# hwang595/ps_pytorch

Measured on AMD Instinct MI355X. Metric: images/sec (whole node), ResNet-18/CIFAR-10 synchronous PS training, higher is better.
Workload: dtype bf16; 1 GPU; model=ResNet18, global_batch=1024, input=3x32x32, per_worker_batch=1024, parallelism=single-gpu, engine=single-machine trainer (hipGraph-captured step), compress_grad=n/a (no comm at N=1), overlap=n/a (no comm at N=1)

## Files before the change

ps_pytorch_amd/ops/__init__.py:

```python
from __future__ import annotations

import ctypes
import os
from pathlib import Path
from typing import Optional

import torch

_LIB: Optional[ctypes.CDLL] = None
_LIB_ERR: Optional[str] = None

PS_F32 = 0
PS_BF16 = 1

_DTYPE_TAG = {torch.float32: PS_F32, torch.bfloat16: PS_BF16}

F32_SYMBOLS = (
    'ps_conv_fwd_f32', 'ps_conv_dgrad_f32', 'ps_conv_wgrad_f32',
    'ps_conv_bias_grad_f32',
    'ps_maxpool_fwd_f32', 'ps_maxpool_bwd_f32',
    'ps_gavgpool_fwd_f32', 'ps_gavgpool_bwd_f32',
    'ps_softmax_ce_fwd_f32', 'ps_softmax_ce_bwd_f32',
    'ps_ce_metrics_f32', 'ps_softmax_ce_fwd_metrics_f32',
)


def _so_path() -> Path:
    return Path(__file__).resolve().parent / "libps_hip.so"


def _try_load() -> None:
    global _LIB, _LIB_ERR
    if _LIB is not None or _LIB_ERR is not None:
        return
    p = _so_path()
    if not p.exists():
        _LIB_ERR = f"{p} not built (run ps_pytorch_amd.ops.build or __graft_entry__.build())"
        return
    try:
        lib = ctypes.CDLL(str(p))
        lib.ps_fused_sgd.argtypes = [
            ctypes.c_void_p, ctypes.c_void_p, ctypes.c_void_p, ctypes.c_void_p,
            ctypes.c_long, ctypes.c_float, ctypes.c_float, ctypes.c_float,
            ctypes.c_float, ctypes.c_int, ctypes.c_int, ctypes.c_int, ctypes.c_void_p]
        lib.ps_pack_bf16.argtypes = [ctypes.c_void_p, ctypes.c_void_p,
                                     ctypes.c_long, ctypes.c_void_p]
        lib.ps_unpack_bf16.argtypes = [ctypes.c_void_p, ctypes.c_void_p,
                                       ctypes.c_long, ctypes.c_void_p]
        lib.ps_pack_q8.argtypes = [ctypes.c_void_p, ctypes.c_void_p,
                                   ctypes.c_long, ctypes.c_int, ctypes.c_void_p]
        lib.ps_pack_q8_ef.argtypes = [ctypes.c_void_p, ctypes.c_void_p,
                                      ctypes.c_void_p, ctypes.c_long,
                                      ctypes.c_int, ctypes.c_void_p]
        lib.ps_pack_bf16_ef.argtypes = [ctypes.c_void_p, ctypes.c_void_p,
                                        ctypes.c_void_p, ctypes.c_long,
                                        ctypes.c_void_p]
        lib.ps_unpack_q8.argtypes = [ctypes.c_void_p, ctypes.c_void_p,
                                     ctypes.c_long, ctypes.c_int, ctypes.c_void_p]
        lib.ps_acc.argtypes = [ctypes.c_void_p, ctypes.c_void_p,
                               ctypes.c_long, ctypes.c_int, ctypes.c_void_p]
        lib.ps_pack_topk_ef.argtypes = [ctypes.c_void_p] * 3 + [
            ctypes.c_long, ctypes.c_int, ctypes.c_int, ctypes.c_void_p]
        lib.ps_pack_topk_ef.restype = ctypes.c_int
        lib.ps_unpack_topk.argtypes = [ctypes.c_void_p, ctypes.c_void_p,
                                       ctypes.c_long, ctypes.c_int,
                                       ctypes.c_int, ctypes.c_void_p]
        lib.ps_unpack_topk.restype = ctypes.c_int
        lib.ps_fanin_reduce.argtypes = [
            ctypes.c_void_p, ctypes.POINTER(ctypes.c_void_p), ctypes.c_int,
            ctypes.c_int, ctypes.c_int, ctypes.c_long, ctypes.c_void_p]
        lib.ps_fanin_reduce.restype = ctypes.c_int
        lib.ps_fanin_sgd.argtypes = [ctypes.c_void_p] * 3 + [
            ctypes.c_int, ctypes.POINTER(ctypes.c_void_p), ctypes.c_int,
            ctypes.c_int, ctypes.c_int, ctypes.c_long] + [
            ctypes.c_float] * 4 + [ctypes.c_int, ctypes.c_void_p]
        lib.ps_fanin_sgd.restype = ctypes.c_int
        lib.ps_conv_fwd.argtypes = [ctypes.c_void_p] * 5 + [ctypes.c_int] * 11 + [ctypes.c_void_p]
        lib.ps_conv_dgrad.argtypes = [ctypes.c_void_p] * 4 + [ctypes.c_int] * 11 + [ctypes.c_void_p]
        lib.ps_conv_wgrad.argtypes = [ctypes.c_void_p] * 4 + [ctypes.c_int] * 12 + [ctypes.c_void_p]
        lib.ps_conv_bias_grad.argtypes = [ctypes.c_void_p] * 3 + [
            ctypes.c_long, ctypes.c_int, ctypes.c_void_p]
        lib.ps_wt_transpose.argtypes = [ctypes.c_void_p, ctypes.c_void_p,
                                        ctypes.c_int, ctypes.c_int, ctypes.c_void_p]
        lib.ps_fused_adam.argtypes = [ctypes.c_void_p] * 6 + [
            ctypes.c_long] + [ctypes.c_float] * 7 + [
            ctypes.c_int, ctypes.c_int, ctypes.c_void_p]
        lib.ps_bn_fwd.argtypes = [ctypes.c_void_p] * 13 + [
            ctypes.c_int,
            ctypes.c_long, ctypes.c_long, ctypes.c_float, ctypes.c_float,
            ctypes.c_int, ctypes.c_int, ctypes.c_int, ctypes.c_void_p]
        lib.ps_bn_bwd.argtypes = [ctypes.c_void_p] * 12 + [
            ctypes.c_long, ctypes.c_long, ctypes.c_int, ctypes.c_int,
            ctypes.c_void_p]
        lib.ps_softmax_ce_fwd.argtypes = [ctypes.c_void_p] * 5 + [
            ctypes.c_long, ctypes.c_int, ctypes.c_void_p]
        lib.ps_softmax_ce_bwd.argtypes = [ctypes.c_void_p] * 5 + [
            ctypes.c_long, ctypes.c_int, ctypes.c_void_p]
        lib.ps_ce_metrics.argtypes = [ctypes.c_void_p] * 5 + [
            ctypes.c_long] + [ctypes.c_int] * 6 + [ctypes.c_void_p]
        lib.ps_softmax_ce_fwd_metrics.argtypes = [ctypes.c_void_p] * 7 + [
            ctypes.c_long] + [ctypes.c_int] * 6 + [ctypes.c_void_p]
        lib.ps_maxpool_fwd.argtypes = [ctypes.c_void_p] * 3 + [
            ctypes.c_int] * 10 + [ctypes.c_void_p]
        lib.ps_maxpool_bwd.argtypes = [ctypes.c_void_p] * 3 + [
            ctypes.c_int] * 10 + [ctypes.c_void_p]
        lib.ps_gavgpool_fwd.argtypes = [ctypes.c_void_p] * 2 + [
            ctypes.c_int] * 3 + [ctypes.c_void_p]
        lib.ps_gavgpool_bwd.argtypes = [ctypes.c_void_p] * 2 + [
            ctypes.c_int] * 3 + [ctypes.c_void_p]
        lib.ps_pad4.argtypes = [ctypes.c_void_p, ctypes.c_void_p,
                                ctypes.c_long, ctypes.c_int, ctypes.c_void_p]
        lib.ps_padc.argtypes = [ctypes.c_void_p, ctypes.c_void_p,
                                ctypes.c_long, ctypes.c_int, ctypes.c_int,
                                ctypes.c_void_p]
        lib.ps_act_drop_fwd.argtypes = [ctypes.c_void_p] * 3 + [
            ctypes.c_long, ctypes.c_int, ctypes.c_int, ctypes.c_uint32,
            ctypes.c_float, ctypes.c_uint64, ctypes.c_uint32,
            ctypes.c_void_p, ctypes.c_void_p]
        lib.ps_act_drop_bwd.argtypes = [ctypes.c_void_p] * 3 + [
            ctypes.c_long, ctypes.c_int, ctypes.c_float, ctypes.c_void_p]
        lib.ps_rng_advance.argtypes = [ctypes.c_void_p, ctypes.c_void_p]
        lib.ps_augment_batch.argtypes = [ctypes.c_void_p] * 5 + [
            ctypes.c_long] + [ctypes.c_int] * 7 + [
            ctypes.POINTER(ctypes.c_float), ctypes.POINTER(ctypes.c_float),
            ctypes.c_uint64, ctypes.c_uint32, ctypes.c_void_p,
            ctypes.c_void_p]
        lib.ps_conv_fwd_f32.argtypes = [ctypes.c_void_p] * 4 + [ctypes.c_int] * 11 + [ctypes.c_void_p]
        lib.ps_conv_dgrad_f32.argtypes = [ctypes.c_void_p] * 4 + [ctypes.c_int] * 11 + [ctypes.c_void_p]
        lib.ps_conv_wgrad_f32.argtypes = [ctypes.c_void_p] * 4 + [ctypes.c_int] * 12 + [ctypes.c_void_p]
        lib.ps_conv_bias_grad_f32.argtypes = [ctypes.c_void_p] * 3 + [
            ctypes.c_long, ctypes.c_int, ctypes.c_void_p]
        lib.ps_softmax_ce_fwd_f32.argtypes = lib.ps_softmax_ce_fwd.argtypes
        lib.ps_softmax_ce_bwd_f32.argtypes = lib.ps_softmax_ce_bwd.argtypes
        lib.ps_ce_metrics_f32.argtypes = lib.ps_ce_metrics.argtypes
        lib.ps_softmax_ce_fwd_metrics_f32.argtypes = \
            lib.ps_softmax_ce_fwd_metrics.argtypes
        lib.ps_maxpool_fwd_f32.argtypes = lib.ps_maxpool_fwd.argtypes
        lib.ps_maxpool_bwd_f32.argtypes = lib.ps_maxpool_bwd.argtypes
        lib.ps_gavgpool_fwd_f32.argtypes = lib.ps_gavgpool_fwd.argtypes
        lib.ps_gavgpool_bwd_f32.argtypes = lib.ps_gavgpool_bwd.argtypes
        _LIB = lib
    except OSError as e:
        _LIB_ERR = str(e)


def lib_or_none() -> Optional[ctypes.CDLL]:
    _try_load()
    return _LIB


def require_lib() -> ctypes.CDLL:
    _try_load()
    if _LIB is None:
        raise RuntimeError(
            f"ps_pytorch_amd HIP extension unavailable on a GPU host: {_LIB_ERR}")
    return _LIB


def dtype_tag(dt: torch.dtype) -> int:
    try:
        return _DTYPE_TAG[dt]
    except KeyError:
        raise TypeError(f"unsupported wire/compute dtype {dt}")


def current_stream_ptr() -> int:
    return torch.cuda.current_stream().cuda_stream


from . import functional
```

ps_pytorch_amd/ops/kernels/conv.hip:

```cpp
#include "common.h"
#include <stdlib.h>

typedef __bf16 bf16x8_t __attribute__((ext_vector_type(8)));
typedef unsigned short ushort8_t __attribute__((ext_vector_type(8)));
typedef float f32x4_t __attribute__((ext_vector_type(4)));

#define MFMA_BF16(a, b, c) __builtin_amdgcn_mfma_f32_16x16x32_bf16(a, b, c, 0, 0, 0)

union V16 {
    uint4 u4;
    unsigned short us[8];
    bf16x8_t bv;
};

__device__ __forceinline__ V16 zero16() {
    V16 v; v.u4 = make_uint4(0, 0, 0, 0); return v;
}

template <bool AL>
__device__ __forceinline__ V16 load16(const unsigned short* src, int cc, int Cn) {
    V16 v;
    if constexpr (AL) {
        v.u4 = *(const uint4*)src;
    } else if (cc + 8 <= Cn) {
// ... 932 lines not shown
    long l = (long)(blockIdx.x & 7) * per_xcd + (blockIdx.x >> 3);
    const long nlog = (long)tiles_k * tiles_c * 3 * split;
    if (l >= nlog) return;
    int b = (int)l;
    const int k0 = (b % tiles_k) * TK; b /= tiles_k;
    const int c0 = (b % tiles_c) * 64; b /= tiles_c;
    const int r = b % 3; b /= 3;
    const int sid = b;
    const long rows_total = (long)Nb * P;
    const long row0 = (long)sid * ipr;
    const long row1 = (row0 + ipr < rows_total) ? row0 + ipr : rows_total;

    const int t = threadIdx.x;
    const int cc8 = (t & 7) * 8;
    const int lane = t & 63, wid = t >> 6;
    const int wm = wid >> 1, wn = wid & 1;
    const int fr = lane & 15, fq = lane >> 4;
    f32x4_t acc[3][MI][2];
#pragma unroll
    for (int s = 0; s < 3; ++s)
#pragma unroll
        for (int i = 0; i < MI; ++i)
#pragma unroll
            for (int j = 0; j < 2; ++j) acc[s][i][j] = {0.f, 0.f, 0.f, 0.f};

    const int nsteps = (int)((row1 - row0 + (1 << (5 - l2q)) - 1)
                             >> (5 - l2q));

    const unsigned short* pdout = dout + (row0 << l2q) * K + k0 + cc8;
    const long inrow0 = row0 + r - PAD;
    const unsigned short* pin = in + inrow0 * W * C + c0 + cc8;
    long prow = row0;

    const int nbq = ROWS * HW2;
    int tb_rib[5], tb_j[5];
    bool tb_ex[5];
    bool tb_v[5];
    long tb_off[5];
#pragma unroll
    for (int u = 0; u < 5; ++u) {
        int idx = (t >> 3) + 32 * u;
        tb_ex[u] = idx < nbq;
        int ix = tb_ex[u] ? idx : 0;
        tb_rib[u] = ix / HW2; tb_j[u] = ix % HW2;
        int wpx = tb_j[u] - 1;
        tb_v[u] = tb_ex[u] && wpx >= 0 && wpx < W;
        tb_off[u] = ((long)tb_rib[u] * W + (wpx < 0 ? 0 : wpx)) * C;
    }
    V16 aregs[TK / 64], bregs[5];

    auto load_step = [&]() {
        bool mrow_ok = (prow + ((t >> 3) >> l2q)) < rows_total;
#pragma unroll
        for (int h = 0; h < TK / 64; ++h)
            aregs[h] = mrow_ok
                ? load16<AL>(pdout + (long)(t >> 3) * K + h * 64,
                             k0 + h * 64 + cc8, K)
                : zero16();
#pragma unroll
        for (int u = 0; u < 5; ++u) {
            int rib = tb_rib[u];
            int p = (int)((prow + rib) & (P - 1));
            int h = p + r - PAD;
            bool v = tb_v[u] && h >= 0 && h < H
                     && (prow + rib) < rows_total;
            bregs[u] = v ? load16<AL>(pin + tb_off[u], c0 + cc8, C)
                         : zero16();
        }
        pdout += (long)32 * K;
        pin += (long)ROWS * W * C;
        prow += ROWS;
    };

    constexpr unsigned A1 = sizeof(lds.A[0]);
    constexpr unsigned BB1 = sizeof(lds.B[0]);
    unsigned short* wrA[TK / 64];
#pragma unroll
    for (int h = 0; h < TK / 64; ++h) {
        int kk8 = h * 64 + cc8;
        wrA[h] = &lds.A[0][kk8 >> 4][pswz(t >> 3) * 16 + (kk8 & 15)];
    }
    unsigned short* wrB[5];
#pragma unroll
    for (int u = 0; u < 5; ++u) {
        int hp = pswz(tb_rib[u] * HW2 + tb_j[u]);
        wrB[u] = &lds.B[0][cc8 >> 4][hp * 16 + (cc8 & 15)];
    }

    auto write_lds = [&](int buf) {
#pragma unroll
        for (int h = 0; h < TK / 64; ++h)
            *(uint4*)((char*)wrA[h] + (buf ? A1 : 0)) = aregs[h].u4;
#pragma unroll
        for (int u = 0; u < 5; ++u)
            if (tb_ex[u])
                *(uint4*)((char*)wrB[u] + (buf ? BB1 : 0)) = bregs[u].u4;
    };

    const char* lb = (const char*)&lds;
    unsigned roA[MI][2];
    unsigned roB[3][2][2];
#pragma unroll
    for (int i = 0; i < 2; ++i) {
        int e = fq * 8 + i * 4 + (fr >> 2);
        int qo = (fr & 3) * 4;
#pragma unroll
        for (int mi = 0; mi < MI; ++mi)
            roA[mi][i] = (unsigned)((char*)&lds.A[0][wm * MI + mi]
                                    [pswz(e) * 16 + qo] - lb);
        int rib = e >> l2q, q = e & (Q - 1);
#pragma unroll
        for (int s = 0; s < 3; ++s) {
            int hp = pswz(rib * HW2 + q + s);
#pragma unroll
            for (int nj = 0; nj < 2; ++nj)
                roB[s][nj][i] = (unsigned)((char*)&lds.B[0][wn * 2 + nj]
                                           [hp * 16 + qo] - lb);
        }
    }

    union U64x8 { bf16x4_t h[2]; bf16x8_t v; };
    auto mfma_step = [&](int buf) {
        U64x8 a[MI];
#pragma unroll
        for (int mi = 0; mi < MI; ++mi) {
            a[mi].h[0] = ds_tr16p((const unsigned short*)
                (lb + roA[mi][0] + (buf ? A1 : 0)));
            a[mi].h[1] = ds_tr16p((const unsigned short*)
                (lb + roA[mi][1] + (buf ? A1 : 0)));
        }
#pragma unroll
        for (int s = 0; s < 3; ++s) {
            U64x8 bf[2];
#pragma unroll
            for (int nj = 0; nj < 2; ++nj) {
                bf[nj].h[0] = ds_tr16p((const unsigned short*)
                    (lb + roB[s][nj][0] + (buf ? BB1 : 0)));
                bf[nj].h[1] = ds_tr16p((const unsigned short*)
                    (lb + roB[s][nj][1] + (buf ? BB1 : 0)));
            }
#pragma unroll
            for (int mi = 0; mi < MI; ++mi)
#pragma unroll
                for (int nj = 0; nj < 2; ++nj)
                    acc[s][mi][nj] = MFMA_BF16(a[mi].v, bf[nj].v,
                                               acc[s][mi][nj]);
        }
    };

    load_step();
    write_lds(0);
    if (nsteps > 1) load_step();
    __syncthreads();
    for (int it = 0; it < nsteps; it += 2) {
        if (it + 1 < nsteps) {
            write_lds(1);
            if (it + 2 < nsteps) load_step();
        }
        mfma_step(0);
        __syncthreads();
        if (it + 1 >= nsteps) break;
        if (it + 2 < nsteps) {
            write_lds(0);
            if (it + 3 < nsteps) load_step();
        }
        mfma_step(1);
        __syncthreads();
    }

    const int RSC = 9 * C;
    float* dstp = partial + (long)sid * K * RSC;
#pragma unroll
    for (int s = 0; s < 3; ++s)
#pragma unroll
    for (int mi = 0; mi < MI; ++mi)
#pragma unroll
    for (int nj = 0; nj < 2; ++nj)
#pragma unroll
    for (int e = 0; e < 4; ++e) {
        int k = k0 + wm * (MI * 16) + mi * 16 + fq * 4 + e;
        int c = c0 + wn * 32 + nj * 16 + fr;
        if (k < K && c < C)
            dstp[(long)k * RSC + (r * 3 + s) * C + c] = acc[s][mi][nj][e];
    }
}


__device__ __forceinline__ int wrho(int e) {
    return (((e >> 1) & 1) + ((e >> 3) & 1) * 2) << 1;
}

template <bool AL>
__global__ __launch_bounds__(256) void conv_wgrad_row_glds_kernel(
    const unsigned short* __restrict__ dout,
    const unsigned short* __restrict__ in,
    float* __restrict__ partial,
    const unsigned short* __restrict__ zpage,
    int Nb, int H, int W, int C, int K, int P, int Q,
    int split, int ipr, int l2q, int l2p, int per_xcd)
{
    constexpr int TK = 64;
    constexpr int PAD = 1;
    const int ROWS = 32 >> l2q;
    const int HW2 = W + 2;
    __shared__ __attribute__((aligned(16))) struct {
        unsigned short A[2][32][64];
        unsigned short B[2][64][64];
    } lds;
    constexpr unsigned A1 = sizeof(lds.A[0]);
    constexpr unsigned BB1 = sizeof(lds.B[0]);
    constexpr int MI = TK / 32;
    const int tiles_k = (K + TK - 1) / TK;
    const int tiles_c = (C + 63) >> 6;
    long l = (long)(blockIdx.x & 7) * per_xcd + (blockIdx.x >> 3);
    const long nlog = (long)tiles_k * tiles_c * 3 * split;
    if (l >= nlog) return;
    int b = (int)l;
    const int k0 = (b % tiles_k) * TK; b /= tiles_k;
    const int c0 = (b % tiles_c) * 64; b /= tiles_c;
    const int r = b % 3; b /= 3;
    const int sid = b;
    const long rows_total = (long)Nb * P;
    const long row0 = (long)sid * ipr;
    const long row1 = (row0 + ipr < rows_total) ? row0 + ipr : rows_total;

    const int t = threadIdx.x;
    const int lane = t & 63, wid = t >> 6;
    const int wm = wid >> 1, wn = wid & 1;
    const int fr = lane & 15, fq = lane >> 4;
    f32x4_t acc[3][MI][2];
#pragma unroll
    for (int si = 0; si < 3; ++si)
#pragma unroll
        for (int i = 0; i < MI; ++i)
#pragma unroll
            for (int j = 0; j < 2; ++j) acc[si][i][j] = {0.f, 0.f, 0.f, 0.f};

    const int nsteps = (int)((row1 - row0 + (1 << (5 - l2q)) - 1)
                             >> (5 - l2q));

    const int apix = wid * 8 + (lane >> 3);
    const int aoct = ((lane & 7) ^ wrho(apix));
    const unsigned short* pdout = dout + (row0 << l2q) * K + k0
                                  + (long)apix * K + aoct * 8;
    const long inrow0 = row0 + r - PAD;
    const unsigned short* pin0 = in + inrow0 * W * C + c0;
    int b_rib[2], b_w[2], b_oct[2];
    bool b_wok[2];
#pragma unroll
    for (int j = 0; j < 2; ++j) {
        int hp = wid * 16 + j * 8 + (lane >> 3);
        b_oct[j] = ((lane & 7) ^ wrho(hp));
        b_rib[j] = hp / HW2;
        int wpx = hp - b_rib[j] * HW2 - 1;
        b_wok[j] = wpx >= 0 && wpx < W && hp < ROWS * HW2;
        b_w[j] = wpx < 0 ? 0 : wpx;
    }
    long prow = row0;

    auto glds_stage = [&](int buf) {
        {
            bool ok = (prow + (apix >> l2q)) < rows_total && apix < 32;
            const unsigned short* gsrc = ok ? pdout : zpage;
            __builtin_amdgcn_global_load_lds(
                (const __attribute__((address_space(1))) void*)gsrc,
                (__attribute__((address_space(3))) void*)
                    &lds.A[buf][wid * 8][0], 16, 0, 0);
        }
#pragma unroll
        for (int j = 0; j < 2; ++j) {
            int rib = b_rib[j];
            int p = (int)((prow + rib) & (P - 1));
            int h = p + r - PAD;
            bool ok = b_wok[j] && h >= 0 && h < H
                      && (prow + rib) < rows_total;
            const unsigned short* gsrc = ok
                ? pin0 + ((long)rib * W + b_w[j]) * C + b_oct[j] * 8
                : zpage;
            __builtin_amdgcn_global_load_lds(
                (const __attribute__((address_space(1))) void*)gsrc,
                (__attribute__((address_space(3))) void*)
                    &lds.B[buf][wid * 16 + j * 8][0], 16, 0, 0);
        }
        pdout += (long)32 * K;
        pin0 += (long)ROWS * W * C;
        prow += ROWS;
    };

    const char* lb0 = (const char*)&lds;
    unsigned roA[MI][2];
    unsigned roB[3][2][2];
#pragma unroll
    for (int i = 0; i < 2; ++i) {
        int e = fq * 8 + i * 4 + (fr >> 2);
        int qd = fr & 3;
#pragma unroll
        for (int mi = 0; mi < MI; ++mi) {
            int o = (wm * MI + mi) * 2 + (qd >> 1);
            roA[mi][i] = (unsigned)((char*)&lds.A[0][e]
                             [(o ^ wrho(e)) * 8 + (qd & 1) * 4] - lb0);
        }
        int rib = e >> l2q, q = e & (Q - 1);
#pragma unroll
        for (int si = 0; si < 3; ++si) {
            int hp = rib * HW2 + q + si;
#pragma unroll
            for (int nj = 0; nj < 2; ++nj) {
                int o = (wn * 2 + nj) * 2 + (qd >> 1);
                roB[si][nj][i] = (unsigned)((char*)&lds.B[0][hp]
                                 [(o ^ wrho(hp)) * 8 + (qd & 1) * 4] - lb0);
            }
        }
    }

    union U64x8 { bf16x4_t h[2]; bf16x8_t v; };
    auto mfma_step = [&](int buf) {
        U64x8 a[MI];
#pragma unroll
        for (int mi = 0; mi < MI; ++mi) {
            a[mi].h[0] = ds_tr16p((const unsigned short*)
                (lb0 + roA[mi][0] + (buf ? A1 : 0)));
            a[mi].h[1] = ds_tr16p((const unsigned short*)
                (lb0 + roA[mi][1] + (buf ? A1 : 0)));
        }
#pragma unroll
        for (int si = 0; si < 3; ++si) {
            U64x8 bf[2];
#pragma unroll
            for (int nj = 0; nj < 2; ++nj) {
                bf[nj].h[0] = ds_tr16p((const unsigned short*)
                    (lb0 + roB[si][nj][0] + (buf ? BB1 : 0)));
                bf[nj].h[1] = ds_tr16p((const unsigned short*)
                    (lb0 + roB[si][nj][1] + (buf ? BB1 : 0)));
            }
#pragma unroll
            for (int mi = 0; mi < MI; ++mi)
#pragma unroll
                for (int nj = 0; nj < 2; ++nj)
                    acc[si][mi][nj] = MFMA_BF16(a[mi].v, bf[nj].v,
                                                acc[si][mi][nj]);
        }
    };

    glds_stage(0);
    __syncthreads();
    for (int it = 0; it < nsteps; ++it) {
        if (it + 1 < nsteps)
            glds_stage((it + 1) & 1);
        mfma_step(it & 1);
        __syncthreads();
    }

    const int RSC = 9 * C;
    float* dstp = partial + (long)sid * K * RSC;
#pragma unroll
    for (int si = 0; si < 3; ++si)
#pragma unroll
    for (int mi = 0; mi < MI; ++mi)
#pragma unroll
    for (int nj = 0; nj < 2; ++nj)
#pragma unroll
    for (int e = 0; e < 4; ++e) {
        int k = k0 + wm * (MI * 16) + mi * 16 + fq * 4 + e;
        int c = c0 + wn * 32 + nj * 16 + fr;
        if (k < K && c < C)
            dstp[(long)k * RSC + (r * 3 + si) * C + c] = acc[si][mi][nj][e];
    }
}

template <int STRIDE, bool POW2, bool AL = true, int CPM = 0>
__global__ __launch_bounds__(256) void conv_wgrad_small_kernel(
    const unsigned short* __restrict__ dout,
    const unsigned short* __restrict__ in,
    float* __restrict__ partial,
    int Nb, int H, int W, int C, int K, int P, int Q,
    int R, int S, int pad, int split, int chunk,
    int l2pq, int l2q,
    unsigned long long mpq, unsigned long long mq)
{
    __shared__ __attribute__((aligned(16))) WgradLds<64> lds;
    const long M = (long)Nb * P * Q;
    const int RSC = R * S * C;
    const int tiles_k = (K + 63) >> 6;
    const int nc = (RSC + 63) >> 6;
    int b = blockIdx.x;
    const int k0 = (b % tiles_k) * 64; b /= tiles_k;
    const int e0 = (b % nc) * 64; b /= nc;
    const int sid = b;
    const long mbeg = (long)sid * chunk;
    const long mend = (mbeg + chunk < M) ? mbeg + chunk : M;

    const int t = threadIdx.x;
    const int trow = t >> 3;
    const int cc8 = (t & 7) * 8;
    const int lane = t & 63, wid = t >> 6;
    const int wm = wid >> 1, wn = wid & 1;
    const int fr = lane & 15, fq = lane >> 4;
    f32x4_t acc[2][2];
#pragma unroll
    for (int i = 0; i < 2; ++i)
#pragma unroll
        for (int j = 0; j < 2; ++j) acc[i][j] = {0.f, 0.f, 0.f, 0.f};

    int tre[8], tse[8], toff[8];
#pragma unroll
    for (int u = 0; u < 8; ++u) {
        int e = e0 + cc8 + u;
        if constexpr (CPM == 8) {
            int tp = e / C;
            tre[u] = tp / S;
            tse[u] = tp - tre[u] * S;
            toff[u] = (tre[u] * W + tse[u]) * C + (e - tp * C);
        } else if constexpr (CPM == 4) {
            int tp = e >> 2;
            tre[u] = tp / S;
            tse[u] = tp - tre[u] * S;
            toff[u] = (tre[u] * W + tse[u]) * 4;
        } else {
            tre[u] = e / (S * C);
            tse[u] = (e / C) % S;
            toff[u] = (tre[u] * W + tse[u]) * C + e % C;
        }
    }

    const int nsteps = (int)((mend - mbeg + 63) >> 6);
    long lm = mbeg;
    V16 areg[2], breg[2];

    auto load_step = [&]() {
#pragma unroll
        for (int rr = 0; rr < 2; ++rr) {
            long m = lm + trow + 32 * rr;
            V16 av = zero16(), bv = zero16();
            if (m < mend) {
                int n, p, q;
                if constexpr (POW2) {
                    n = (int)(m >> l2pq);
                    int rem = (int)m & ((1 << l2pq) - 1);
                    p = rem >> l2q; q = rem & ((1 << l2q) - 1);
                } else {
                    n = (int)fdiv_u32((unsigned)m, mpq);
                    unsigned rem = (unsigned)m - (unsigned)n * (unsigned)(P * Q);
                    p = (int)fdiv_u32(rem, mq);
                    q = (int)(rem - (unsigned)p * (unsigned)Q);
                }
                av = load16<AL>(dout + m * K + k0 + cc8, k0 + cc8, K);
                int h0 = p * STRIDE - pad, w0 = q * STRIDE - pad;
                const unsigned short* pix =
                    in + (long)n * H * W * C + ((long)h0 * W + w0) * C;
                if constexpr (CPM == 8) {
                    int hh = h0 + tre[0], ww = w0 + tse[0];
                    if (e0 + cc8 < RSC
                        && hh >= 0 && hh < H && ww >= 0 && ww < W)
                        bv.u4 = *(const uint4*)(pix + toff[0]);
                } else if constexpr (CPM == 4) {
#pragma unroll
                    for (int half = 0; half < 2; ++half) {
                        int u = 4 * half;
                        int hh = h0 + tre[u], ww = w0 + tse[u];
                        if (e0 + cc8 + u < RSC
                            && hh >= 0 && hh < H && ww >= 0 && ww < W)
                            *(unsigned long long*)&bv.us[u] =
                                *(const unsigned long long*)(pix + toff[u]);
                    }
                } else {
#pragma unroll
                for (int u = 0; u < 8; ++u) {
                    int hh = h0 + tre[u], ww = w0 + tse[u];
                    if (e0 + cc8 + u < RSC
                        && hh >= 0 && hh < H && ww >= 0 && ww < W)
                        bv.us[u] = pix[toff[u]];
                }
                }
            }
            areg[rr] = av; breg[rr] = bv;
        }
        lm += 64;
    };

    constexpr unsigned A1 = 4 * WG_SUB * 2;
    constexpr unsigned BB1 = A1;
    unsigned short* wrA[2];
    unsigned short* wrB[2];
#pragma unroll
    for (int rr = 0; rr < 2; ++rr) {
        int midx = pswz(trow + 32 * rr);
        wrA[rr] = &lds.A[0][cc8 >> 4][midx * 16 + (cc8 & 15)];
        wrB[rr] = &lds.B[0][cc8 >> 4][midx * 16 + (cc8 & 15)];
    }
    unsigned roA[2][2][2];
    unsigned roB[2][2][2];
#pragma unroll
    for (int kk = 0; kk < 2; ++kk)
#pragma unroll
        for (int i = 0; i < 2; ++i) {
            int m = pswz(kk * 32 + fq * 8 + i * 4 + (fr >> 2));
            int qo = (fr & 3) * 4;
#pragma unroll
            for (int mi = 0; mi < 2; ++mi)
                roA[kk][mi][i] = (unsigned)((char*)&lds.A[0][wm * 2 + mi]
                                            [m * 16 + qo] - (char*)&lds);
#pragma unroll
            for (int nj = 0; nj < 2; ++nj)
// ... 316 lines not shown
        int Nout_ = DG ? C : K;                                               \
        long grid = ((M_ + TM - 1) / TM) * ((Nout_ + TN - 1) / TN);           \
        hipLaunchKernelGGL((conv_gemm_kernel<TM, TN, ST, DG, SM, ALV, NBV,    \
                                             SWV, ACV, 0, GLV, STV>),         \
            dim3((unsigned)grid), dim3(256), 0, (hipStream_t)strm,            \
            (const unsigned short*)src, (const unsigned short*)wgt,           \
            (const unsigned short*)bias, (unsigned short*)dst,                \
            (const unsigned short*)carry, zpage_ptr(), (float*)stats,         \
            Nb, H, W, C, K, P, Q, R, S, pad);                                 \
    } while (0)
#define LAUNCH_GEMM_GL(TM, TN, ST, DG, SM, NBV, SWV, ACV, GLV)                \
    do {                                                                      \
        if (!(DG) && stats) LAUNCH_GEMM_GLS(TM, TN, ST, DG, SM, NBV, SWV, ACV, GLV, true); \
        else                LAUNCH_GEMM_GLS(TM, TN, ST, DG, SM, NBV, SWV, ACV, GLV, false); \
    } while (0)
#define LAUNCH_GEMM_SW(TM, TN, ST, DG, SM, NBV, SWV, ACV)                     \
    do {                                                                      \
        if constexpr (ALV && !(SM)) {                                         \
            if (glds_mode()) LAUNCH_GEMM_GL(TM, TN, ST, DG, SM, NBV, SWV, ACV, true); \
            else             LAUNCH_GEMM_GL(TM, TN, ST, DG, SM, NBV, SWV, ACV, false); \
        } else {                                                              \
            LAUNCH_GEMM_GL(TM, TN, ST, DG, SM, NBV, SWV, ACV, false);         \
        }                                                                     \
    } while (0)

extern "C" void ps_conv_fwd(
    const void* src, const void* wgt, const void* bias, void* dst,
    void* stats,
    int Nb, int H, int W, int C, int K, int P, int Q,
    int R, int S, int stride, int pad, void* strm)
{
    const void* carry = nullptr;
    bool al = (C & 63) == 0;
#define FWD_BODY()                                                            \
    do {                                                                      \
        if (R * S > 1 && C == 4 && R * S * 4 <= 64) {        \
            if (K <= 32) {            \
                if (stride == 1) LAUNCH_GEMM_CV(128, 32, 1, true, 1);         \
                else             LAUNCH_GEMM_CV(128, 32, 2, true, 1);         \
            } else if (stride == 1) LAUNCH_GEMM_CV(128, 64, 1, true, 1);      \
            else             LAUNCH_GEMM_CV(128, 64, 2, true, 1);             \
        } else if (R * S > 1 && C == 4 && R * S * 4 <= 256) {                 \
            if (K <= 32) {                                                    \
                if (stride == 1) LAUNCH_GEMM_CV(128, 32, 1, true, 2);         \
                else             LAUNCH_GEMM_CV(128, 32, 2, true, 2);         \
            } else if (stride == 1) LAUNCH_GEMM_CV(128, 64, 1, true, 2);      \
            else             LAUNCH_GEMM_CV(128, 64, 2, true, 2);             \
        } else if (R * S > 1 && (C & 7) == 0 && (C & 63)                      \
                   && R * S * C <= 768) {              \
            if (K <= 32) {                                                    \
                if (stride == 1) LAUNCH_GEMM_CP(128, 32, 1, true, 2, 8);      \
                else             LAUNCH_GEMM_CP(128, 32, 2, true, 2, 8);      \
            } else if (stride == 1) LAUNCH_GEMM_CP(128, 64, 1, true, 2, 8);   \
            else             LAUNCH_GEMM_CP(128, 64, 2, true, 2, 8);          \
        } else if (R * S > 1 && R * S * C <= 64) {    \
            if (stride == 1) LAUNCH_GEMM_NB(128, 64, 1, false, true, 1);      \
            else             LAUNCH_GEMM_NB(128, 64, 2, false, true, 1);      \
        } else if (R * S > 1 && R * S * C <= 192) {                           \
            if (stride == 1) LAUNCH_GEMM(128, 64, 1, false, true);            \
            else             LAUNCH_GEMM(128, 64, 2, false, true);            \
        } else if (R * S == 1 && C <= 64) {              \
            if (stride == 1) LAUNCH_GEMM_NB(128, 64, 1, false, false, 1);     \
            else             LAUNCH_GEMM_NB(128, 64, 2, false, false, 1);     \
        } else if (K >= 128) {                                                \
            if (stride == 1) LAUNCH_GEMM(128, 128, 1, false, false);          \
            else             LAUNCH_GEMM(128, 128, 2, false, false);          \
        } else if (K <= 32) {         \
            if (stride == 1) LAUNCH_GEMM(128, 32, 1, false, false);           \
            else             LAUNCH_GEMM(128, 32, 2, false, false);           \
        } else {                                                              \
            if (stride == 1) LAUNCH_GEMM(128, 64, 1, false, false);           \
            else             LAUNCH_GEMM(128, 64, 2, false, false);           \
        }                                                                     \
    } while (0)
    if (al) { constexpr bool ALV = true; FWD_BODY(); }
    else    { constexpr bool ALV = false; FWD_BODY(); }
#undef FWD_BODY
}

extern "C" void ps_conv_dgrad(
    const void* src, const void* wgt, void* dst, const void* carry,
    int Nb, int H, int W, int C, int K, int P, int Q,
    int R, int S, int stride, int pad, void* strm)
{
    const void* bias = nullptr;
    const void* stats = nullptr;
    bool al = (K & 63) == 0;
    if (stride == 1) {
#define DG_BODY(ACV)                                                          \
        do {                                                                  \
            if (C >= 128)     LAUNCH_GEMM_ACC(128, 128, 1, true, false, ACV); \
            else if (C <= 32) LAUNCH_GEMM_ACC(128, 32, 1, true, false, ACV);  \
            else              LAUNCH_GEMM_ACC(128, 64, 1, true, false, ACV);  \
        } while (0)
        if (al) { constexpr bool ALV = true;
                  if (carry) DG_BODY(true); else DG_BODY(false); }
        else    { constexpr bool ALV = false;
                  if (carry) DG_BODY(true); else DG_BODY(false); }
#undef DG_BODY
    } else {
        const unsigned short* dout = (const unsigned short*)src;
        bool any_empty = false;
        for (int hp = 0; hp < 2 && hp < H; ++hp)
        for (int wp = 0; wp < 2 && wp < W; ++wp) {
            int r0 = (hp + pad) & 1, s0 = (wp + pad) & 1;
            if (R <= r0 || S <= s0) any_empty = true;
        }
        if (any_empty)
            launch_seed_dx(dst, carry, (long)Nb * H * W * C, strm);
        int TM_ = 128, TN_ = (C >= 128) ? 128 : 64;
        int tiles_n_ = (C + TN_ - 1) / TN_;
        int ends_[4] = {0, 0, 0, 0}, codes_[4] = {0, 0, 0, 0};
        int slot = 0, total = 0;
        for (int hp = 0; hp < 2 && hp < H; ++hp)
        for (int wp = 0; wp < 2 && wp < W; ++wp) {
            int r0 = (hp + pad) & 1, s0 = (wp + pad) & 1;
            if (R <= r0 || S <= s0) continue;
            int Hc = (H - hp + 1) >> 1, Wc = (W - wp + 1) >> 1;
            long M_ = (long)Nb * Hc * Wc;
            total += (int)(((M_ + TM_ - 1) / TM_) * tiles_n_);
            ends_[slot] = total;
            codes_[slot] = (hp << 1) | wp;
            ++slot;
        }
        for (int i = slot; i < 4; ++i) { ends_[i] = total; codes_[i] = 0; }
        if (total == 0) return;
        int4 ends = make_int4(ends_[0], ends_[1], ends_[2], ends_[3]);
        int4 codes = make_int4(codes_[0], codes_[1], codes_[2], codes_[3]);
#define DG2_SW(TM, TN, ALV, SWV, ACV)                                         \
        hipLaunchKernelGGL((conv_dgrad2_kernel<TM, TN, ALV, SWV, ACV>),       \
            dim3((unsigned)total), dim3(256), 0, (hipStream_t)strm, dout,     \
            (const unsigned short*)wgt, (unsigned short*)dst,                 \
            (const unsigned short*)carry,                                     \
            Nb, H, W, C, K, P, Q, R, S, pad, ends, codes)
#define DG2_AC(TM, TN, ALV, SWV) do {                                         \
        if (carry) DG2_SW(TM, TN, ALV, SWV, true);                            \
        else       DG2_SW(TM, TN, ALV, SWV, false); } while (0)
#define DG2(TM, TN, ALV) do {                                                 \
        if (swz_mode() == 1) DG2_AC(TM, TN, ALV, 1);                          \
        else                 DG2_AC(TM, TN, ALV, 2); } while (0)
        if (al) { if (C >= 128) DG2(128, 128, true);
                  else          DG2(128, 64, true); }
        else    { if (C >= 128) DG2(128, 128, false);
                  else          DG2(128, 64, false); }
#undef DG2
    }
}

static inline int ilog2_exact(long v) {
    int l = 0; while ((1L << l) < v) ++l;
    return ((1L << l) == v) ? l : -1;
}

extern "C" void ps_conv_wgrad(
    const void* dout, const void* in, void* partial_f32, void* dw,
    int Nb, int H, int W, int C, int K, int P, int Q,
    int R, int S, int stride, int pad, int split, void* strm)
{
    long M = (long)Nb * P * Q;
    long chunk64 = (M + (long)split * 64 - 1) / ((long)split * 64);
    int chunk = (int)(chunk64 * 64);
    if (R * S > 1 && ((C == 4 && R * S * 4 <= 256)
                      || ((C & 7) == 0 && (C & 63) && R * S * C <= 768)
                      || R * S * C <= 192)) {
        int tiles_k = (K + 63) / 64;
        int nc_s = (R * S * C + 63) / 64;
        long grid_s = (long)tiles_k * nc_s * split;
        int l2pq_ = ilog2_exact((long)P * Q), l2q_ = ilog2_exact(Q);
        bool pw = l2pq_ >= 0 && l2q_ >= 0;
        unsigned long long mpq_ = fdiv_magic((long)P * Q);
        unsigned long long mq_ = fdiv_magic(Q);
#define WGS(ST, PW, CV)                                                       \
        hipLaunchKernelGGL((conv_wgrad_small_kernel<ST, PW, false, CV>),      \
            dim3((unsigned)grid_s), dim3(256), 0, (hipStream_t)strm,          \
            (const unsigned short*)dout, (const unsigned short*)in,           \
            (float*)partial_f32, Nb, H, W, C, K, P, Q, R, S, pad, split,      \
            chunk, l2pq_, l2q_, mpq_, mq_)
        if (C == 4) {
            if (stride == 1) { if (pw) WGS(1, true, 4); else WGS(1, false, 4); }
            else             { if (pw) WGS(2, true, 4); else WGS(2, false, 4); }
        } else if ((C & 7) == 0 && (C & 63)) {
            if (stride == 1) { if (pw) WGS(1, true, 8); else WGS(1, false, 8); }
            else             { if (pw) WGS(2, true, 8); else WGS(2, false, 8); }
        } else {
            if (stride == 1) { if (pw) WGS(1, true, 0); else WGS(1, false, 0); }
            else             { if (pw) WGS(2, true, 0); else WGS(2, false, 0); }
        }
#undef WGS
        long n_ = (long)K * R * S * C;
        launch_reduce_slabs((unsigned short*)dw, (float*)partial_f32, n_,
                            split, (hipStream_t)strm);
        return;
    }
    {
        static int row_en = -1;
        if (row_en < 0) row_en = getenv("PS_WG_ROW_OFF") ? 0 : 1;
        int l2q_ = ilog2_exact(Q), l2pq_ = ilog2_exact((long)P * Q);
        if (row_en && stride == 1 && R == 3 && S == 3 && pad == 1 && P == H
            && Q == W && l2q_ >= 0 && l2pq_ >= 0 && Q >= 4 && Q <= 32) {
            static int wg_glds = -1;
            if (wg_glds < 0) {
                const char* e = getenv("PS_WG_GLDS");
                wg_glds = e ? atoi(e) : 0;
            }
            const int TKr = 64;
            int tkr = (K + TKr - 1) / TKr, tcr = (C + 63) / 64;
            long rows_total = (long)Nb * P;
            int ROWS = 32 >> l2q_;
            long ipr_l = (rows_total + split - 1) / split;
            ipr_l = ((ipr_l + ROWS - 1) / ROWS) * ROWS;
            long nlog = (long)tkr * tcr * 3 * split;
            int pxc = (int)((nlog + 7) / 8);
            long grid_r = (long)pxc * 8;
            bool alr = ((C & 63) == 0) && (K % TKr == 0);
#define WGR(TKV, ALV)                                                         \
            hipLaunchKernelGGL((conv_wgrad_row_kernel<TKV, ALV>),             \
                dim3((unsigned)grid_r), dim3(256), 0, (hipStream_t)strm,      \
                (const unsigned short*)dout, (const unsigned short*)in,       \
                (float*)partial_f32, Nb, H, W, C, K, P, Q,                    \
                split, (int)ipr_l, l2q_, 0, pxc)
#define WGRG(ALV)                                                             \
            hipLaunchKernelGGL((conv_wgrad_row_glds_kernel<ALV>),             \
                dim3((unsigned)grid_r), dim3(256), 0, (hipStream_t)strm,      \
                (const unsigned short*)dout, (const unsigned short*)in,       \
                (float*)partial_f32, zpage_ptr(), Nb, H, W, C, K, P, Q,       \
                split, (int)ipr_l, l2q_, 0, pxc)
            if (wg_glds && alr) WGRG(true);
            else if (alr)       WGR(64, true);
            else                WGR(64, false);
#undef WGRG
#undef WGR
            long n_ = (long)K * 9 * C;
            launch_reduce_slabs((unsigned short*)dw, (float*)partial_f32, n_,
                                split, (hipStream_t)strm);
            return;
        }
    }
    int TK = (K >= 128) ? 128 : 64;
    int tiles_k = (K + TK - 1) / TK, tiles_c = (C + 63) / 64;
    long nlog = (long)tiles_k * tiles_c * R * S * split;
    int per_xcd = (int)((nlog + 7) / 8);
    long grid = (long)per_xcd * 8;
    int l2pq = ilog2_exact((long)P * Q), l2q = ilog2_exact(Q);
    bool pow2 = l2pq >= 0 && l2q >= 0;
    unsigned long long mpq = fdiv_magic((long)P * Q);
    unsigned long long mq = fdiv_magic(Q);
#define WG_LAUNCH(ST, PW, TKV)                                                \
    hipLaunchKernelGGL((conv_wgrad_kernel<ST, PW, TKV, ALV>),                 \
        dim3((unsigned)grid), dim3(256), 0, (hipStream_t)strm,                \
        (const unsigned short*)dout, (const unsigned short*)in,               \
        (float*)partial_f32, Nb, H, W, C, K, P, Q, R, S, pad, split, chunk,   \
        l2pq, l2q, per_xcd, mpq, mq)
#define WG_TK(ST, PW) do { if (TK == 128) WG_LAUNCH(ST, PW, 128);             \
                           else WG_LAUNCH(ST, PW, 64); } while (0)
#define WG_AL(ST, PW) do { if ((C & 63) == 0 && K % TK == 0) {                \
        constexpr bool ALV = true; WG_TK(ST, PW);                             \
    } else { constexpr bool ALV = false; WG_TK(ST, PW); } } while (0)
    if (stride == 1) { if (pow2) WG_AL(1, true); else WG_AL(1, false); }
    else             { if (pow2) WG_AL(2, true); else WG_AL(2, false); }
#undef WG_AL
#undef WG_TK
#undef WG_LAUNCH
    long n = (long)K * R * S * C;
    launch_reduce_slabs((unsigned short*)dw, (float*)partial_f32, n, split,
                        (hipStream_t)strm);
}

extern "C" void ps_conv_bias_grad(
    void* db, const void* dout, void* partial_f32, long M, int K, void* strm)
{
    int nblk = (int)((M + 3) / 4 < 512 ? (M + 3) / 4 : 512);
    hipLaunchKernelGGL(colsum_part_kernel, dim3(nblk), dim3(256), 0,
                       (hipStream_t)strm, (float*)partial_f32,
                       (const unsigned short*)dout, M, K);
    hipLaunchKernelGGL(colsum_fold_kernel, dim3(K), dim3(256), 0,
                       (hipStream_t)strm, (unsigned short*)db,
                       (const float*)partial_f32, nblk, K);
}

__global__ __launch_bounds__(256) void wt_transpose_kernel(
    const unsigned short* __restrict__ w, unsigned short* __restrict__ wt,
    int K, int RSC)
{
    __shared__ unsigned short tile[32][33];
    int tiles_e = (RSC + 31) >> 5;
    int k0 = (blockIdx.x / tiles_e) << 5;
    int e0 = (blockIdx.x % tiles_e) << 5;
    int tx = threadIdx.x & 31, ty = threadIdx.x >> 5;
#pragma unroll
    for (int i = 0; i < 4; ++i) {
        int k = k0 + ty + 8 * i, e = e0 + tx;
        tile[ty + 8 * i][tx] =
            (k < K && e < RSC) ? w[(long)k * RSC + e] : (unsigned short)0;
    }
    __syncthreads();
#pragma unroll
    for (int i = 0; i < 4; ++i) {
        int e = e0 + ty + 8 * i, k = k0 + tx;
        if (e < RSC && k < K)
            wt[(long)e * K + k] = tile[tx][ty + 8 * i];
    }
}

extern "C" void ps_wt_transpose(void* wt, const void* w, int K, int RSC,
                                void* strm)
{
    long grid = (long)((K + 31) / 32) * ((RSC + 31) / 32);
    hipLaunchKernelGGL(wt_transpose_kernel, dim3((unsigned)grid), dim3(256), 0,
                       (hipStream_t)strm, (const unsigned short*)w,
                       (unsigned short*)wt, K, RSC);
}
```

Measured before the change: 113,100 images/sec.

## Replace double-buffered global-to-LDS wgrad row kernel with 4-stage ring pipeline

Replaces the opt-in double-buffered global_load_lds wgrad row kernel with a ring-buffered variant that keeps up to three stages of direct-to-LDS DMA in flight. It uses inline asm for the m0-based loads and partial vmcnt waits, and makes this ring kernel the default for aligned 3x3 stride-1 wgrad. It also peels the tail of the register-staged row kernel's main loop so the steady-state loop has no branches. The goal is to hide global memory latency behind MFMA work in the weight-gradient convolutions. In exchange it uses more LDS per block, which may lower occupancy, and it relies on hand-written asm wait counts being correct.

New measurement: 129,300 images/sec (median of 6 runs). +14.3%, better.

```diff
diff --git a/ps_pytorch_amd/ops/__init__.py b/ps_pytorch_amd/ops/__init__.py
--- a/ps_pytorch_amd/ops/__init__.py
+++ b/ps_pytorch_amd/ops/__init__.py
@@ -78,6 +78,9 @@
         lib.ps_conv_fwd.argtypes = [ctypes.c_void_p] * 5 + [ctypes.c_int] * 11 + [ctypes.c_void_p]
         lib.ps_conv_dgrad.argtypes = [ctypes.c_void_p] * 4 + [ctypes.c_int] * 11 + [ctypes.c_void_p]
         lib.ps_conv_wgrad.argtypes = [ctypes.c_void_p] * 4 + [ctypes.c_int] * 12 + [ctypes.c_void_p]
+        lib.ps_conv_wgrad_row_variant.argtypes = [ctypes.c_void_p] * 3 + [
+            ctypes.c_int] * 9 + [ctypes.c_void_p]
+        lib.ps_conv_wgrad_row_variant.restype = ctypes.c_int
         lib.ps_conv_bias_grad.argtypes = [ctypes.c_void_p] * 3 + [
             ctypes.c_long, ctypes.c_int, ctypes.c_void_p]
         lib.ps_wt_transpose.argtypes = [ctypes.c_void_p, ctypes.c_void_p,
diff --git a/ps_pytorch_amd/ops/kernels/conv.hip b/ps_pytorch_amd/ops/kernels/conv.hip
--- a/ps_pytorch_amd/ops/kernels/conv.hip
+++ b/ps_pytorch_amd/ops/kernels/conv.hip
@@ -1108,20 +1108,31 @@
     write_lds(0);
     if (nsteps > 1) load_step();
     __syncthreads();
-    for (int it = 0; it < nsteps; it += 2) {
-        if (it + 1 < nsteps) {
-            write_lds(1);
-            if (it + 2 < nsteps) load_step();
-        }
+    int it = 0;
+    for (; it + 3 < nsteps; it += 2) {
+        write_lds(1);
+        load_step();
         mfma_step(0);
         __syncthreads();
-        if (it + 1 >= nsteps) break;
-        if (it + 2 < nsteps) {
-            write_lds(0);
-            if (it + 3 < nsteps) load_step();
-        }
+        write_lds(0);
+        load_step();
         mfma_step(1);
         __syncthreads();
+    }
+    const int rem = nsteps - it;
+    if (rem >= 2) {
+        write_lds(1);
+        if (rem >= 3) load_step();
+    }
+    if (rem >= 1) mfma_step(0);
+    if (rem >= 2) {
+        __syncthreads();
+        if (rem >= 3) write_lds(0);
+        mfma_step(1);
+    }
+    if (rem >= 3) {
+        __syncthreads();
+        mfma_step(0);
     }
 
     const int RSC = 9 * C;
@@ -1146,8 +1157,37 @@
     return (((e >> 1) & 1) + ((e >> 3) & 1) * 2) << 1;
 }
 
-template <bool AL>
-__global__ __launch_bounds__(256) void conv_wgrad_row_glds_kernel(
+#define WG_RING_NST 4
+
+struct WgRingStage {
+    unsigned short A[32][64];
+    unsigned short B[64][64];
+};
+
+__device__ __forceinline__ void wg_ring_dma3(
+    const void* g0, const void* g1, const void* g2,
+    unsigned l0, unsigned l1, unsigned l2)
+{
+    unsigned keep;
+    asm volatile(
+        "s_mov_b32 %0, m0\n\t"
+        "s_mov_b32 m0, %4\n\ts_nop 0\n\tglobal_load_lds_dwordx4 %1, off\n\t"
+        "s_mov_b32 m0, %5\n\ts_nop 0\n\tglobal_load_lds_dwordx4 %2, off\n\t"
+        "s_mov_b32 m0, %6\n\ts_nop 0\n\tglobal_load_lds_dwordx4 %3, off\n\t"
+        "s_mov_b32 m0, %0"
+        : "=&s"(keep)
+        : "v"(g0), "v"(g1), "v"(g2), "s"(l0), "s"(l1), "s"(l2)
+        : "memory");
+}
+
+template <int N>
+__device__ __forceinline__ void wg_ring_sync() {
+    asm volatile("s_waitcnt vmcnt(%0)\n\ts_waitcnt lgkmcnt(0)\n\ts_barrier"
+                 :: "i"(N) : "memory");
+}
+
+template <int NST>
+__global__ __launch_bounds__(256) void conv_wgrad_row_ring_kernel(
     const unsigned short* __restrict__ dout,
     const unsigned short* __restrict__ in,
     float* __restrict__ partial,
@@ -1155,16 +1195,16 @@
     int Nb, int H, int W, int C, int K, int P, int Q,
     int split, int ipr, int l2q, int l2p, int per_xcd)
 {
+    static_assert(NST == 3 || NST == 4, "ring depth");
     constexpr int TK = 64;
     constexpr int PAD = 1;
+    constexpr int DPS = 3;
     const int ROWS = 32 >> l2q;
     const int HW2 = W + 2;
-    __shared__ __attribute__((aligned(16))) struct {
-        unsigned short A[2][32][64];
-        unsigned short B[2][64][64];
-    } lds;
-    constexpr unsigned A1 = sizeof(lds.A[0]);
-    constexpr unsigned BB1 = sizeof(lds.B[0]);
+    __shared__ __attribute__((aligned(16))) WgRingStage sg0, sg1, sg2, sg3;
+    auto stg = [&](int st) -> WgRingStage* {
+        return st == 0 ? &sg0 : st == 1 ? &sg1 : st == 2 ? &sg2 : &sg3;
+    };
     constexpr int MI = TK / 32;
     const int tiles_k = (K + TK - 1) / TK;
     const int tiles_c = (C + 63) >> 6;
@@ -1197,53 +1237,51 @@
 
     const int apix = wid * 8 + (lane >> 3);
     const int aoct = ((lane & 7) ^ wrho(apix));
-    const unsigned short* pdout = dout + (row0 << l2q) * K + k0
-                                  + (long)apix * K + aoct * 8;
+    const unsigned short* pdout = dout + (row0 << l2q) * K + k0;
+    const int a_off = apix * K + aoct * 8;
+    const int a_row = apix >> l2q;
     const long inrow0 = row0 + r - PAD;
     const unsigned short* pin0 = in + inrow0 * W * C + c0;
-    int b_rib[2], b_w[2], b_oct[2];
+    int b_rib[2], b_off[2];
     bool b_wok[2];
 #pragma unroll
     for (int j = 0; j < 2; ++j) {
         int hp = wid * 16 + j * 8 + (lane >> 3);
-        b_oct[j] = ((lane & 7) ^ wrho(hp));
+        int oct = ((lane & 7) ^ wrho(hp));
         b_rib[j] = hp / HW2;
         int wpx = hp - b_rib[j] * HW2 - 1;
         b_wok[j] = wpx >= 0 && wpx < W && hp < ROWS * HW2;
-        b_w[j] = wpx < 0 ? 0 : wpx;
+        b_off[j] = (b_rib[j] * W + (wpx < 0 ? 0 : wpx)) * C + oct * 8;
     }
     long prow = row0;
 
-    auto glds_stage = [&](int buf) {
-        {
-            bool ok = (prow + (apix >> l2q)) < rows_total && apix < 32;
-            const unsigned short* gsrc = ok ? pdout : zpage;
-            __builtin_amdgcn_global_load_lds(
-                (const __attribute__((address_space(1))) void*)gsrc,
-                (__attribute__((address_space(3))) void*)
-                    &lds.A[buf][wid * 8][0], 16, 0, 0);
-        }
+    const unsigned wu = (unsigned)__builtin_amdgcn_readfirstlane(wid);
+    const unsigned ldA = wu * (8 * 128);
+    const unsigned ldB = (unsigned)sizeof(sg0.A) + wu * (16 * 128);
+
+    auto dma_stage = [&](int st) {
+        const unsigned sb = (unsigned)(unsigned long)
+            (__attribute__((address_space(3))) void*)stg(st);
+        const unsigned short* gs[DPS];
+        const long rl = rows_total - prow;
+        const int rleft = rl < 64 ? (int)rl : 64;
+        const int pl = (int)prow;
+        gs[0] = a_row < rleft ? pdout + a_off : zpage;
 #pragma unroll
         for (int j = 0; j < 2; ++j) {
-            int rib = b_rib[j];
-            int p = (int)((prow + rib) & (P - 1));
-            int h = p + r - PAD;
-            bool ok = b_wok[j] && h >= 0 && h < H
-                      && (prow + rib) < rows_total;
-            const unsigned short* gsrc = ok
-                ? pin0 + ((long)rib * W + b_w[j]) * C + b_oct[j] * 8
-                : zpage;
-            __builtin_amdgcn_global_load_lds(
-                (const __attribute__((address_space(1))) void*)gsrc,
-                (__attribute__((address_space(3))) void*)
-                    &lds.B[buf][wid * 16 + j * 8][0], 16, 0, 0);
-        }
+            int h = ((pl + b_rib[j]) & (P - 1)) + r - PAD;
+            bool ok = b_wok[j] & ((unsigned)h < (unsigned)H)
+                      & (b_rib[j] < rleft);
+            gs[1 + j] = ok ? pin0 + b_off[j] : zpage;
+        }
+        wg_ring_dma3(gs[0], gs[1], gs[2],
+                     sb + ldA, sb + ldB, sb + ldB + 8 * 128);
         pdout += (long)32 * K;
         pin0 += (long)ROWS * W * C;
         prow += ROWS;
     };
 
-    const char* lb0 = (const char*)&lds;
+    const char* lb0 = (const char*)&sg0;
     unsigned roA[MI][2];
     unsigned roB[3][2][2];
 #pragma unroll
@@ -1253,7 +1291,7 @@
 #pragma unroll
         for (int mi = 0; mi < MI; ++mi) {
             int o = (wm * MI + mi) * 2 + (qd >> 1);
-            roA[mi][i] = (unsigned)((char*)&lds.A[0][e]
+            roA[mi][i] = (unsigned)((char*)&sg0.A[e]
                              [(o ^ wrho(e)) * 8 + (qd & 1) * 4] - lb0);
         }
         int rib = e >> l2q, q = e & (Q - 1);
@@ -1263,21 +1301,22 @@
 #pragma unroll
             for (int nj = 0; nj < 2; ++nj) {
                 int o = (wn * 2 + nj) * 2 + (qd >> 1);
-                roB[si][nj][i] = (unsigned)((char*)&lds.B[0][hp]
+                roB[si][nj][i] = (unsigned)((char*)&sg0.B[hp]
                                  [(o ^ wrho(hp)) * 8 + (qd & 1) * 4] - lb0);
             }
         }
     }
 
     union U64x8 { bf16x4_t h[2]; bf16x8_t v; };
-    auto mfma_step = [&](int buf) {
+    auto mfma_step = [&](int st) {
+        const char* sbp = (const char*)stg(st);
         U64x8 a[MI];
 #pragma unroll
         for (int mi = 0; mi < MI; ++mi) {
             a[mi].h[0] = ds_tr16p((const unsigned short*)
-                (lb0 + roA[mi][0] + (buf ? A1 : 0)));
+                (sbp + roA[mi][0]));
             a[mi].h[1] = ds_tr16p((const unsigned short*)
-                (lb0 + roA[mi][1] + (buf ? A1 : 0)));
+                (sbp + roA[mi][1]));
         }
 #pragma unroll
         for (int si = 0; si < 3; ++si) {
@@ -1285,9 +1324,9 @@
 #pragma unroll
             for (int nj = 0; nj < 2; ++nj) {
                 bf[nj].h[0] = ds_tr16p((const unsigned short*)
-                    (lb0 + roB[si][nj][0] + (buf ? BB1 : 0)));
+                    (sbp + roB[si][nj][0]));
                 bf[nj].h[1] = ds_tr16p((const unsigned short*)
-                    (lb0 + roB[si][nj][1] + (buf ? BB1 : 0)));
+                    (sbp + roB[si][nj][1]));
             }
 #pragma unroll
             for (int mi = 0; mi < MI; ++mi)
@@ -1298,13 +1337,33 @@
         }
     };
 
-    glds_stage(0);
-    __syncthreads();
-    for (int it = 0; it < nsteps; ++it) {
-        if (it + 1 < nsteps)
-            glds_stage((it + 1) & 1);
-        mfma_step(it & 1);
-        __syncthreads();
+    auto ring_sync = [&](int ahead) {
+        if (NST > 3 && ahead >= 2) wg_ring_sync<2 * DPS>();
+        else if (ahead >= 1)       wg_ring_sync<DPS>();
+        else                       wg_ring_sync<0>();
+    };
+
+#pragma unroll
+    for (int j = 0; j < NST - 1; ++j)
+        if (j < nsteps) dma_stage(j);
+    int it = 0;
+    for (; it + 2 * NST - 2 < nsteps; it += NST) {
+#pragma unroll
+        for (int j = 0; j < NST; ++j) {
+            ring_sync(NST - 2);
+            dma_stage((j + NST - 1) % NST);
+            mfma_step(j);
+        }
+    }
+    const int rem = nsteps - it;
+#pragma unroll
+    for (int j = 0; j < 2 * NST - 2; ++j) {
+        if (j < rem) {
+            const int left = rem - 1 - j;
+            ring_sync(left < NST - 2 ? left : NST - 2);
+            if (j + NST - 1 < rem) dma_stage((j + NST - 1) % NST);
+            mfma_step(j % NST);
+        }
     }
 
     const int RSC = 9 * C;
@@ -1927,6 +1986,62 @@
     return ((1L << l) == v) ? l : -1;
 }
 
+static bool wgrad_row_eligible(int H, int W, int C, int K, int P, int Q,
+                               int variant)
+{
+    if (P != H || Q != W || ilog2_exact(Q) < 0 || ilog2_exact(P) < 0
+        || Q < 4 || Q > 32)
+        return false;
+    if (variant == 1) return (C & 63) == 0 && (K & 63) == 0;
+    return variant == 0;
+}
+
+static void launch_wgrad_row(
+    const void* dout, const void* in, void* partial_f32,
+    int Nb, int H, int W, int C, int K, int P, int Q, int split,
+    int variant, void* strm)
+{
+    const int TKr = 64;
+    int l2q_ = ilog2_exact(Q);
+    int tkr = (K + TKr - 1) / TKr, tcr = (C + 63) / 64;
+    long rows_total = (long)Nb * P;
+    int ROWS = 32 >> l2q_;
+    long ipr_l = (rows_total + split - 1) / split;
+    ipr_l = ((ipr_l + ROWS - 1) / ROWS) * ROWS;
+    long nlog = (long)tkr * tcr * 3 * split;
+    int pxc = (int)((nlog + 7) / 8);
+    long grid_r = (long)pxc * 8;
+    bool alr = ((C & 63) == 0) && (K % TKr == 0);
+#define WGR(TKV, ALV)                                                         \
+    hipLaunchKernelGGL((conv_wgrad_row_kernel<TKV, ALV>),                     \
+        dim3((unsigned)grid_r), dim3(256), 0, (hipStream_t)strm,              \
+        (const unsigned short*)dout, (const unsigned short*)in,               \
+        (float*)partial_f32, Nb, H, W, C, K, P, Q,                            \
+        split, (int)ipr_l, l2q_, 0, pxc)
+    if (variant == 1)
+        hipLaunchKernelGGL((conv_wgrad_row_ring_kernel<WG_RING_NST>),
+            dim3((unsigned)grid_r), dim3(256), 0, (hipStream_t)strm,
+            (const unsigned short*)dout, (const unsigned short*)in,
+            (float*)partial_f32, zpage_ptr(), Nb, H, W, C, K, P, Q,
+            split, (int)ipr_l, l2q_, 0, pxc);
+    else if (alr) WGR(64, true);
+    else          WGR(64, false);
+#undef WGR
+}
+
+extern "C" int ps_conv_wgrad_row_variant(
+    const void* dout, const void* in, void* partial_f32,
+    int Nb, int H, int W, int C, int K, int P, int Q, int split,
+    int variant, void* strm)
+{
+    if (split < 1 || Nb < 1
+        || !wgrad_row_eligible(H, W, C, K, P, Q, variant))
+        return 1;
+    launch_wgrad_row(dout, in, partial_f32, Nb, H, W, C, K, P, Q, split,
+                     variant, strm);
+    return 0;
+}
+
 extern "C" void ps_conv_wgrad(
     const void* dout, const void* in, void* partial_f32, void* dw,
     int Nb, int H, int W, int C, int K, int P, int Q,
@@ -1970,41 +2085,17 @@
     {
         static int row_en = -1;
         if (row_en < 0) row_en = getenv("PS_WG_ROW_OFF") ? 0 : 1;
-        int l2q_ = ilog2_exact(Q), l2pq_ = ilog2_exact((long)P * Q);
-        if (row_en && stride == 1 && R == 3 && S == 3 && pad == 1 && P == H
-            && Q == W && l2q_ >= 0 && l2pq_ >= 0 && Q >= 4 && Q <= 32) {
-            static int wg_glds = -1;
-            if (wg_glds < 0) {
-                const char* e = getenv("PS_WG_GLDS");
-                wg_glds = e ? atoi(e) : 0;
-            }
-            const int TKr = 64;
-            int tkr = (K + TKr - 1) / TKr, tcr = (C + 63) / 64;
-            long rows_total = (long)Nb * P;
-            int ROWS = 32 >> l2q_;
-            long ipr_l = (rows_total + split - 1) / split;
-            ipr_l = ((ipr_l + ROWS - 1) / ROWS) * ROWS;
-            long nlog = (long)tkr * tcr * 3 * split;
-            int pxc = (int)((nlog + 7) / 8);
-            long grid_r = (long)pxc * 8;
-            bool alr = ((C & 63) == 0) && (K % TKr == 0);
-#define WGR(TKV, ALV)                                                         \
-            hipLaunchKernelGGL((conv_wgrad_row_kernel<TKV, ALV>),             \
-                dim3((unsigned)grid_r), dim3(256), 0, (hipStream_t)strm,      \
-                (const unsigned short*)dout, (const unsigned short*)in,       \
-                (float*)partial_f32, Nb, H, W, C, K, P, Q,                    \
-                split, (int)ipr_l, l2q_, 0, pxc)
-#define WGRG(ALV)                                                             \
-            hipLaunchKernelGGL((conv_wgrad_row_glds_kernel<ALV>),             \
-                dim3((unsigned)grid_r), dim3(256), 0, (hipStream_t)strm,      \
-                (const unsigned short*)dout, (const unsigned short*)in,       \
-                (float*)partial_f32, zpage_ptr(), Nb, H, W, C, K, P, Q,       \
-                split, (int)ipr_l, l2q_, 0, pxc)
-            if (wg_glds && alr) WGRG(true);
-            else if (alr)       WGR(64, true);
-            else                WGR(64, false);
-#undef WGRG
-#undef WGR
+        if (row_en && stride == 1 && R == 3 && S == 3 && pad == 1
+            && wgrad_row_eligible(H, W, C, K, P, Q, 0)) {
+            static int wg_ring = -1;
+            if (wg_ring < 0) {
+                const char* e = getenv("PS_WG_RING");
+                wg_ring = e ? atoi(e) : 1;
+            }
+            int variant = (wg_ring
+                           && wgrad_row_eligible(H, W, C, K, P, Q, 1)) ? 1 : 0;
+            launch_wgrad_row(dout, in, partial_f32, Nb, H, W, C, K, P, Q,
+                             split, variant, strm);
             long n_ = (long)K * 9 * C;
             launch_reduce_slabs((unsigned short*)dw, (float*)partial_f32, n_,
                                 split, (hipStream_t)strm);
```
